# Fireflies-17/Speech-Inpainting

Hardware: AMD Instinct MI355X
Metric: real-time factor (audio-sec/wall-sec) per GPU, 4 s clips @16 kHz, 200 ms mask (higher is better)
Workload: dtype encoder GEMMs and attention products: bf16 MFMA, fp32 accumulate (softmax, LayerNorm, head, arg-max in fp32); vocoder: fp16 MFMA (operands rounded to fp16, saturating), fp32 accumulate, activations stored as fp16; 1 GPU; BASELINE configs[1]: batch=32 x 4 s clips per GPU, 200 ms mask, HuBERT-base + HiFi-GAN V1; step = masked log-mel front-end -> encoder -> arg-max/splice -> vocoder on resident raw clips; global_batch=32, clip_samples=64000, mask_frames=10, parallelism=utterance-sharded x1

## Files before the change

include/si_hip.h:

```cpp
#ifndef SI_HIP_H
#define SI_HIP_H

#include <stddef.h>
#include <stdint.h>

#ifdef __cplusplus
extern "C" {
#endif

#define SI_ABI_VERSION 3

enum {
    SI_OK = 0,
    SI_EINVAL = -1,
    SI_ENOMEM = -2,
    SI_EHIP = -3,
    SI_ESTATE = -4,
    SI_EWEIGHTS = -5
};

enum {
    SI_MATH_F32 = 0,
    SI_MATH_BF16 = 1,
    SI_MATH_BF16X3 = 2,
// ... 118 lines not shown
    const double* dwin;
    const double* time_reg;
} si_sinc_filter;
int si_resample_sinc(si_ctx* ctx, const float* x, const int32_t* n_len, int B, int n_in, const si_sinc_filter* f, int n_out, float* y,
                     si_stream_t stream);

int si_pcm16(si_ctx* ctx, const float* wav, int64_t n, int16_t* out, si_stream_t stream);

int si_hifigan_forward(si_ctx* ctx, const float* mel, int B, int Tm, int stretch, float* wav_out,
                       void* workspace, size_t workspace_bytes, si_stream_t stream);

int si_extend_mel(si_ctx* ctx, const float* mel, int B, int Tm, float* out, si_stream_t stream);

int si_hifigan_forward_varlen(si_ctx* ctx, const float* mel, const int32_t* mel_len, int B, int Tm, int stretch, float* wav_out,
                              void* workspace, size_t workspace_bytes, si_stream_t stream);

int si_mel_frames(int n22);
int si_mel_workspace_bytes(si_ctx* ctx, int B, int N22, size_t* out);
int si_mel_frontend(si_ctx* ctx, const float* wave22, const int32_t* mask_start, const int32_t* mask_end, int normalize,
                    int B, int N22, float* mel_out, void* workspace, size_t workspace_bytes, si_stream_t stream);

int si_mel_frontend_varlen(si_ctx* ctx, const float* wave22, const int32_t* mask_start, const int32_t* mask_end, const int32_t* sample_len,
                           int normalize, int B, int N22, float* mel_out, void* workspace, size_t workspace_bytes, si_stream_t stream);

#define SI_MAX_SPANS 16
typedef struct si_span_table {
    int32_t struct_size;
    int32_t num_clips;
    int32_t num_spans;
    int32_t reserved;
// ... 151 lines not shown
```

speech_inpainting_amd/csrc/api.hip:

```cpp
#include <cmath>
#include <cstdarg>
#include <cstdio>
#include <cstdlib>
#include <cstring>
#include <map>
#include <sstream>
#include <string>
#include <vector>

#include "common.h"

namespace {

struct HostTensor {
    const float* data = nullptr;
    std::vector<long> shape;
    long numel() const { long n = 1; for (long d : shape) n *= d; return n; }
};

struct GemmW {
    size_t w = 0, w_lo = 0, bias = 0;
    int Cin = 0, N = 0, Npad = 0, ntaps = 0, groups = 1, math = 0;
    bool has_bias = false;
};

struct LayerW { GemmW qkv, out, ffn1, ffn2; size_t ln1_g, ln1_b, ln2_g, ln2_b; };
struct ConvW { GemmW g; size_t ln_g = 0, ln_b = 0; };
struct ResW { GemmW c1[SI_MAX_DIL], c2[SI_MAX_DIL]; };

struct Layout {
    size_t total = 0;
    size_t conv0_w, conv0_bias, conv0_g, conv0_b;
    std::vector<ConvW> convs;
    size_t fp_ln_g, fp_ln_b; GemmW proj;
    GemmW pos; size_t enc_ln_g, enc_ln_b;
    std::vector<LayerW> layers;
// ... 209 lines not shown
    L.cb_rnorm = P.floats(d.num_clusters);
    L.mel_ld = si_round_up(d.num_mels, 32);
    const int C0 = d.up_initial_channel;
    L.pre = P.gemm(vm, 1, 7, C0, L.mel_ld, true);
    L.ups.clear(); L.rbs.clear();
    int c = C0;
    for (int i = 0; i < d.num_ups; ++i) {
        const int u = d.up_rates[i], k = d.up_kernels[i], cout = stage_channels(ctx, i);
        L.ups.push_back(P.gemm(vm, 1, (k + u - 1) / u, u * cout, c, true));
        c = cout;
        for (int j = 0; j < d.num_rb; ++j) {
            ResW r;
            for (int n = 0; n < d.num_dil; ++n) {
                r.c1[n] = P.gemm(vm, 1, d.rb_kernels[j], c, c, true);
                if (d.resblock_type != 2) r.c2[n] = P.gemm(vm, 1, d.rb_kernels[j], c, c, true);
            }
            L.rbs.push_back(r);
        }
    }
    L.post_C = c;
    L.post_w = P.floats((size_t)7 * c);
    L.post_b = P.floats(1);
    L.total = P.cur;
    return SI_OK;
}

struct BlobHeader { uint32_t magic, version; uint64_t fingerprint, total; uint64_t reserved; };
constexpr uint32_t BLOB_MAGIC = 0x42574953u;
uint64_t layout_fingerprint(const si_ctx* ctx) {
    uint64_t h = 1469598103934665603ull;
// ... 242 lines not shown
        for (int j = 0; j < d.num_rb; ++j) {
            const ResW& R = L.rbs[(size_t)i * d.num_rb + j];
            const std::string rp = G + "resblocks." + std::to_string(i * d.num_rb + j) + ".";
            for (int n = 0; n < d.num_dil; ++n) {
                if (d.resblock_type == 2) {
                    const std::string a = rp + "convs." + std::to_string(n);
                    if (P.folded(a, {c, c, d.rb_kernels[j]}, 0, w)) P.conv(R.c1[n], w, c, c, d.rb_kernels[j]);
                    P.bias(R.c1[n], a + ".bias", c);
                    continue;
                }
                const std::string a = rp + "convs1." + std::to_string(n), bb = rp + "convs2." + std::to_string(n);
                if (P.folded(a, {c, c, d.rb_kernels[j]}, 0, w)) P.conv(R.c1[n], w, c, c, d.rb_kernels[j]);
                P.bias(R.c1[n], a + ".bias", c);
                if (P.folded(bb, {c, c, d.rb_kernels[j]}, 0, w)) P.conv(R.c2[n], w, c, c, d.rb_kernels[j]);
                P.bias(R.c2[n], bb + ".bias", c);
            }
        }
    }
    if (P.folded(G + "conv_post", {1, c, 7}, 0, w))
        for (int ci = 0; ci < c; ++ci) for (int k = 0; k < 7; ++k) P.fptr(L.post_w)[(size_t)k * L.post_C + ci] = w[(size_t)ci * 7 + k];
    P.copy_floats(L.post_b, G + "conv_post.bias", 1);
    return P.rc;
}

inline size_t align_up(size_t v, size_t a) { return (v + a - 1) / a * a; }

struct Carver {
    char* base; size_t cap; size_t cur = 0; bool ok = true;
    float* floats(size_t n) { return reinterpret_cast<float*>(bytes(n * 4)); }
    char* bytes(size_t n) {
// ... 981 lines not shown
                        if (opr) {
                            q.x = nullptr; q.x16 = in16;
                            if (r16) { q.res = nullptr; q.res16 = y16; q.out = nullptr; }
                            if (o.copy16) { q.out16 = ynext16; q.out16_slope = o.slope16; }
                        }
                        q.alpha = o.alpha; q.accumulate = o.accumulate; q.acc16 = r16 && o.accumulate;
                        return si_launch_tapgemm(ctx, G.math, q, st);
                    };
                    if (d.resblock_type == 2) {
                        if ((rc = residual_conv(R.c1[n], dl, in_slope, y, y16))) return rc;
                    } else {
                        int frc = 1;
                        if (r16 && (fuse_mask & cout)) {
                            const TapGemmParams w1 = gemm_params(ctx, R.c1[n]), w2 = gemm_params(ctx, R.c2[n]);
                            frc = si_launch_respair(ctx, cout, y16, ynext16, w1.w, w2.w, w1.bias, w2.bias, Bc, (int)Lo, rk, dl, o.alpha, o.accumulate, st,
                                                    dLs(i + 1), hLs(i + 1), o.slope16);
                            if (frc < 0) return frc;
                        }
                        if (frc > 0) {
                            float* t = buf[3];
                            TapGemmParams p = stage_conv(R.c1[n], i + 1, Lo, cout, cout, dl);
                            p.x = y; p.out = t; p.pro_slope = in_slope;
                            if (opr) { p.x = nullptr; p.x16 = y16; p.out = nullptr; p.out16 = t16; p.out16_slope = 0.1f; }
                            if ((rc = si_launch_tapgemm(ctx, R.c1[n].math, p, st))) return rc;
                            if ((rc = !opr ? tap32({t, nst}, "stage%d.rb%d.t%d", i, j, n)
                                           : tap32({t16, nst, 2}, d.vocoder_math == SI_MATH_F16 ? "stage%d.rb%d.t%d.f16" : "stage%d.rb%d.t%d.bf16", i, j, n))) return rc;
                            if ((rc = residual_conv(R.c2[n], 1, opr ? 1.f : 0.1f, t, t16))) return rc;
                        }
                    }
                    if ((rc = tap16(ynext16, nst, "stage%d.rb%d.p%d.f16", i, j, n))) return rc;
                    if ((rc = tap32({ynext, nst}, "stage%d.rb%d.p%d", i, j, n))) return rc;
// ... 90 lines not shown
    ctx->fe_dev = dev;
    return SI_OK;
}

size_t mel_ws_bytes(int B, int N22) {
    const long Tm = (N22 + 2 * FE_PAD - FE_NFFT) / FE_HOP + 1;
    if (Tm < 1) return 0;
    return fe_round((size_t)B * 4) + fe_round((size_t)B * Tm * FE_FRAME * 4) + fe_round((size_t)B * Tm * FE_LDSPEC * 4) + 256 +
           fe_round((size_t)2 * B * 4);
}

}

extern "C" {

int si_mel_frames(int n22) { return n22 + 2 * FE_PAD < FE_NFFT ? 0 : (n22 + 2 * FE_PAD - FE_NFFT) / FE_HOP + 1; }

int si_mel_workspace_bytes(si_ctx* ctx, int B, int N22, size_t* out) {
    if (!ctx || !out || B <= 0 || si_mel_frames(N22) < 1) return si_fail(ctx, SI_EINVAL, "si_mel_workspace_bytes: bad argument");
    *out = mel_ws_bytes(B, N22);
    return SI_OK;
}

static int mel_run(si_ctx* ctx, const float* wave22, const int32_t* mask_start, const int32_t* mask_end, int normalize, int B,
                   int N22, float* mel_out, void* workspace, size_t workspace_bytes, si_stream_t stream, const int32_t* host_len,
                   const SiSpans* spans = nullptr);

int si_mel_frontend_spans(si_ctx* ctx, const float* wave22, const si_span_table* spans, const int32_t* sample_len, int normalize,
                          int B, int N22, float* mel_out, void* workspace, size_t workspace_bytes, si_stream_t stream) {
    if (!ctx) return SI_EINVAL;
// ... 410 lines not shown
```

speech_inpainting_amd/csrc/common.h:

```cpp
#pragma once
#include <hip/hip_runtime.h>
#include <stdint.h>

#include "../../include/si_hip.h"

#define SI_HIP_CHECK(expr)                                                                      \
    do {                                                                                        \
        hipError_t _e = (expr);                                                                 \
        if (_e != hipSuccess) return si_fail_hip(ctx, _e, #expr, __FILE__, __LINE__);           \
    } while (0)

int si_fail_hip(si_ctx* ctx, hipError_t e, const char* what, const char* file, int line);
int si_fail(si_ctx* ctx, int code, const char* fmt, ...);
void si_prof_begin(si_ctx* ctx, const char* name, double flops, double bytes, hipStream_t st);
void si_prof_end(si_ctx* ctx, hipStream_t st);
const char* si_prof_shape_name(const char* name, long M, int N, int K);
int si_ensure_dyn_lds(si_ctx* ctx, const void* kern, size_t bytes);
int si_num_cus(si_ctx* ctx);

typedef unsigned short bf16_t;

struct SiVlTile { int b, row0, L; };
#ifdef __HIPCC__
__device__ __forceinline__ SiVlTile si_vl_tile(const int32_t* __restrict__ lens, int B, int step, int t) {
// ... 264 lines not shown
int si_launch_upsample_stream(si_ctx* ctx, const UpsampleParams& p, hipStream_t st);

struct ResPairParams {
    const unsigned short* y16;
    unsigned short* out16;
    const unsigned short* w1;
    const unsigned short* w2;
    const float* b1;
    const float* b2;
    int B, L, k, dil;
    float alpha;
    int accumulate;
    const int32_t* lens; const int32_t* lens_host;
    int total_tiles;
    float out_slope;
};
int si_launch_respair_wide(si_ctx* ctx, int C, const ResPairParams& p, hipStream_t st);
struct ResChainParams {
    const unsigned short* y16;
    unsigned short* out16;
    const unsigned short* w1[3];
    const unsigned short* w2[3];
    const float* b1[3];
    const float* b2[3];
    int B, L, k;
    int dil[3];
    float alpha;
    int accumulate;
    const int32_t* lens; const int32_t* lens_host;
    int total_tiles;
};
int si_launch_reschain(si_ctx* ctx, int C, const ResChainParams& p, hipStream_t st);
int si_launch_respair(si_ctx* ctx, int C, const unsigned short* y16, unsigned short* out16, const void* w1, const void* w2,
                      const float* b1, const float* b2, int B, int L, int k, int dil, float alpha, int accumulate, hipStream_t st,
                      const int32_t* lens = nullptr, const int32_t* lens_host = nullptr, float out_slope = 1.f);

int si_launch_extend_mel(si_ctx* ctx, const float* mel, int B, int D, int Tm, int Tout, int stretch, float* out, int ldo,
                         hipStream_t st, const int32_t* tm_len = nullptr, const int32_t* tout_len = nullptr);
int si_launch_extend_mel_cf(si_ctx* ctx, const float* mel, int B, int D, int Tm, int Tout, float* out, hipStream_t st);
int si_launch_small_conv1d(si_ctx* ctx, const float* x, const float* w, const float* bias, const float* res, float* y, int B, int Cin,
                           int Tin, int Cout, int Tout, int K, int stride, int dil, int pad, int relu_in, int channels_last, hipStream_t st);
int si_launch_f0enc_fused(si_ctx* ctx, const float* weights, const float* f0, int B, int T, float* h_out, int in_width, int out_width, int width,
                          int n_state, int depth, int down_t, int stride_t, int growth, int dk, int dpad, double macs, hipStream_t st);
int si_launch_unit_frontend(si_ctx* ctx, const int64_t* code, int Fc, const int64_t* f0_code, int Fp, const float* spk_emb,
                            const float* emb_c, int Kc, const float* emb_p, int Kp, int E, int B, float* out, hipStream_t st);
int si_launch_conv_post(si_ctx* ctx, const float* x, const float* w , const float* bias, int B, int L, int C, int k,
                        float* wav, hipStream_t st, const unsigned short* x16 = nullptr ,
                        const int32_t* lens = nullptr, const int32_t* lens_host = nullptr);
```

speech_inpainting_amd/csrc/respair.hip:

```cpp
#include <algorithm>
#include <cstdio>
#include <cstdlib>
#include <type_traits>

#include "common.h"

typedef float f32x4 __attribute__((ext_vector_type(4)));
typedef unsigned int u32x4 __attribute__((ext_vector_type(4)));
typedef unsigned int u32x2 __attribute__((ext_vector_type(2)));
typedef _Float16 f16x8 __attribute__((ext_vector_type(8)));
typedef _Float16 f16x4 __attribute__((ext_vector_type(4)));

constexpr int RPN_HALO = 50;

template <int ROWB>
__device__ __forceinline__ int rpn_swz(int row) {
    if constexpr (ROWB == 128) return (row & 7) << 4;
    else return ((row >> 1) & 3) << 4;
}

template <int C, int R1, int WARPS_M, int TPS, bool ACC, bool VL>
__global__ __launch_bounds__(64 * WARPS_M, 2) void respair_kernel(const ResPairParams p) {
    static_assert(R1 == WARPS_M * 64 && (C == 32 || C == 64), "64-row wave tiles over all C channels");
    constexpr int NT = 64 * WARPS_M;
// ... 264 lines not shown
    const int grid = std::min(total, si_num_cus(ctx) * (WARPS_M == 4 ? 2 : 1));
    char name[48];
    snprintf(name, sizeof(name), p.accumulate ? "respair_f16_c%d_acc" : "respair_f16_c%d", C);
    double rows = (double)p.B * p.L;
    if (vl) { rows = 0; for (int b = 0; b < p.B; ++b) rows += p.lens_host[b]; }
    const double elems = rows * C;
    si_prof_begin(ctx, name, 2.0 * 2.0 * elems * C * p.k, elems * (2.0 + 2.0 + (p.accumulate ? 2.0 : 0.0)) + 2.0 * 2.0 * p.k * C * C, st);
    hipLaunchKernelGGL(kern, dim3(grid), dim3(64 * WARPS_M), lds, st, pk);
    si_prof_end(ctx, st);
    SI_HIP_CHECK(hipGetLastError());
    return SI_OK;
}

int si_launch_respair(si_ctx* ctx, int C, const unsigned short* y16, unsigned short* out16, const void* w1, const void* w2,
                      const float* b1, const float* b2, int B, int L, int k, int dil, float alpha, int accumulate, hipStream_t st,
                      const int32_t* lens, const int32_t* lens_host, float out_slope) {
    if ((C != 32 && C != 64 && C != 128 && C != 256) || k < 3 || k > 11 || (k & 1) == 0 || (k - 1) * dil > 50 ||
        ((long)L + 1024) * C * 2 >= (1L << 31)) return 1;
    if (!b1 || !b2) return 1;
    if ((lens == nullptr) != (lens_host == nullptr)) return si_fail(ctx, SI_EINVAL, "respair: ragged batches need the lengths on the device and on the host");
    ResPairParams p{y16, out16, static_cast<const unsigned short*>(w1), static_cast<const unsigned short*>(w2), b1, b2, B, L, k, dil, alpha, accumulate, lens, lens_host, 0, out_slope};
    if (out_slope != 1.f && C < 128) return 1;
    if (C >= 128) return si_launch_respair_wide(ctx, C, p, st);
    return C == 32 ? respair_launch<32, 256, 4, 11>(ctx, p, st) : respair_launch<64, 512, 8, 4>(ctx, p, st);
}
```

speech_inpainting_amd/csrc/respair_wide.hip:

```cpp
#include <algorithm>
#include <cstdio>
#include <cstdlib>

#include "common.h"

typedef float f32x4 __attribute__((ext_vector_type(4)));
typedef unsigned int u32x4 __attribute__((ext_vector_type(4)));
typedef unsigned int u32x2 __attribute__((ext_vector_type(2)));
typedef _Float16 f16x8 __attribute__((ext_vector_type(8)));
typedef _Float16 f16x4 __attribute__((ext_vector_type(4)));

template <int ROWB>
__device__ __forceinline__ int swz16(int row) {
    if constexpr (ROWB >= 256) return (row & 7) << 5;
    else return ((row >> 1) & 3) << 5;
}

#ifdef RPW_TIMELINE
__device__ unsigned long long rpw_tl[2][10];
#define RPW_TL_DECL unsigned long long tl_t = wall_clock64(); unsigned long long tl_acc[6] = {0, 0, 0, 0, 0, 0}; unsigned long long tl_tiles = 0; unsigned long long tl_w = 0, tl_sub[2] = {0, 0};
#define RPW_TL_W0 tl_w = wall_clock64();
#define RPW_TL_W1(q) tl_sub[q] += wall_clock64() - tl_w;
#define RPW_TL(ph) { const unsigned long long n_ = wall_clock64(); tl_acc[ph] += n_ - tl_t; tl_t = n_; }
#define RPW_TL_TILE ++tl_tiles;
// ... 1 lines not shown
extern "C" int si_debug_rpw_timeline(unsigned long long* out, int reset) {
    if (hipMemcpyFromSymbol(out, HIP_SYMBOL(rpw_tl), sizeof(rpw_tl)) != hipSuccess) return -1;
    if (reset) { unsigned long long z[2][10] = {}; if (hipMemcpyToSymbol(HIP_SYMBOL(rpw_tl), z, sizeof(z)) != hipSuccess) return -1; }
    return 0;
}
#else
#define RPW_TL_DECL
#define RPW_TL_W0
#define RPW_TL_W1(q)
#define RPW_TL(ph)
#define RPW_TL_TILE
#define RPW_TL_FLUSH
#endif

constexpr int RPW_HALO = 50;

template <int C, int R1, int WARPS_M, int WARPS_N, int BKW, bool ACC, bool VL>
__global__ __launch_bounds__(64 * WARPS_M * WARPS_N, 2) void respair_wide_kernel(const ResPairParams p) {
    static_assert((WARPS_M * WARPS_N == 8 || WARPS_M * WARPS_N == 4) && R1 == WARPS_M * 64 && C == WARPS_N * 64, "64 x 64 wave tiles");
    static_assert(BKW == 128 || BKW == 64, "weight-slab depth");
    constexpr int NT = 64 * WARPS_M * WARPS_N;
    constexpr int ROWBY = C * 2;
    constexpr int ROWBW = BKW * 2;
    constexpr int ROWBO = C * 4;
    constexpr int CPRY = C / 8, CPRW = BKW / 8;
    constexpr int NCH = C / BKW;
    constexpr int KS = BKW / 32;
    constexpr int YBYTES = (R1 + RPW_HALO) * ROWBY;
    constexpr int WBYTES = C * ROWBW;
    constexpr int WSLOTS = C * CPRW / NT;
    constexpr int YSLOTS = ((R1 + RPW_HALO) * CPRY + NT - 1) / NT;
    constexpr int YRPP = NT / CPRY, WRPP = NT / CPRW;
    static_assert(C * CPRW % NT == 0 && NT % CPRY == 0 && NT % CPRW == 0, "staging maps");
    static_assert(R1 * ROWBO <= YBYTES + 2 * WBYTES, "the output image reuses the operand region (not the biases behind it)");

    __builtin_amdgcn_s_setreg((0 << 11) | (23 << 6) | 1, 1);
    extern __shared__ __attribute__((aligned(16))) char smem[];
    char* const Ys = smem;
    char* const Ws = smem + YBYTES;
    float* const Bs = reinterpret_cast<float*>(smem + YBYTES + 2 * WBYTES);

    const int tid = threadIdx.x, lane = tid & 63, wave = tid >> 6;
    const int r16 = lane & 15, kg = lane >> 4;
    const int wm0 = (wave / WARPS_N) * 64, wn0 = (wave % WARPS_N) * 64;
    const int k = p.k, d = p.dil;
    const int p1 = d * (k - 1) / 2, p2 = (k - 1) / 2;
    const int BMo = R1 - (k - 1);
    const int R0 = R1 + (k - 1) * d;
    const int tiles_x = (p.L + BMo - 1) / BMo;
    const int total = VL ? p.total_tiles : tiles_x * p.B;
    auto tile_of = [&](int t, int& tb, int& tm0, int& tL) {
        if constexpr (VL) { const SiVlTile v = si_vl_tile(p.lens, p.B, BMo, t); tb = v.b; tm0 = v.row0; tL = v.L; }
        else { tb = t / tiles_x; tm0 = (t - tb * tiles_x) * BMo; tL = p.L; }
    };
    const __amdgpu_buffer_rsrc_t w1rsrc = __builtin_amdgcn_make_buffer_rsrc(const_cast<unsigned short*>(p.w1), 0, k * C * C * 2, 0x00020000);
    const __amdgpu_buffer_rsrc_t w2rsrc = __builtin_amdgcn_make_buffer_rsrc(const_cast<unsigned short*>(p.w2), 0, k * C * C * 2, 0x00020000);

    const int NS1 = k * NCH, NS = 2 * NS1;
    const int wc = tid % CPRW, wr0 = tid / CPRW;
    u32x4 rw[WSLOTS];
    auto issueW1 = [&](int s, int i) {
        const bool second = s >= NS1;
        const int q = second ? s - NS1 : s;
        const int tap = q / NCH, ch = q - tap * NCH;
        const int soff = __builtin_amdgcn_readfirstlane((tap * C * C + ch * BKW) * 2);
        const int n = wr0 + i * WRPP;
        rw[i] = __builtin_amdgcn_raw_buffer_load_b128(second ? w2rsrc : w1rsrc, (n * C + 8 * wc) * 2, soff, 0);
    };
    auto issueW = [&](int s) {
#pragma unroll
        for (int i = 0; i < WSLOTS; ++i) issueW1(s, i);
    };
    auto storeW1 = [&](char* dst, int i) {
        const int n = wr0 + i * WRPP;
        *reinterpret_cast<u32x4*>(dst + n * ROWBW + ((wc << 4) ^ swz16<ROWBW>(n))) = rw[i];
    };
    auto storeW = [&](char* dst) {
#pragma unroll
        for (int i = 0; i < WSLOTS; ++i) storeW1(dst, i);
    };
    const int yc = tid % CPRY, yr0 = tid / CPRY;
    u32x4 ry[YSLOTS];
    auto issueY = [&](int t) {
        int tb, tm0, tL;
        tile_of(t, tb, tm0, tL);
        const int trow0 = tm0 - p2 - p1;
        const __amdgpu_buffer_rsrc_t rs = __builtin_amdgcn_make_buffer_rsrc(const_cast<unsigned short*>(p.y16 + (long)tb * p.L * C), 0, tL * C * 2, 0x00020000);
#pragma unroll
        for (int i = 0; i < YSLOTS; ++i)
            ry[i] = __builtin_amdgcn_raw_buffer_load_b128(rs, ((trow0 + yr0 + i * YRPP) * C + 8 * yc) * 2, 0, 0);
    };

    if (tid < C / 2) {
        const int which = tid / (C / 4), c4 = (tid % (C / 4)) * 4;
        *reinterpret_cast<f32x4*>(Bs + which * C + c4) = *reinterpret_cast<const f32x4*>((which ? p.b2 : p.b1) + c4);
    }
    const int preW = (wn0 + r16) * ROWBW + (swz16<ROWBW>(wn0 + r16) ^ (kg << 4));
    issueW(0);
    issueY(blockIdx.x);
    RPW_TL_DECL

  for (int tile = blockIdx.x; tile < total; tile += gridDim.x) {
    const int nxt = tile + (int)gridDim.x < total ? tile + (int)gridDim.x : tile;
    int b, m0, Lb;
    tile_of(tile, b, m0, Lb);
    const int t_row0 = m0 - p2;
    const long seg = (long)b * p.L * C;
    const __amdgpu_buffer_rsrc_t yrsrc = __builtin_amdgcn_make_buffer_rsrc(const_cast<unsigned short*>(p.y16 + seg), 0, Lb * C * 2, 0x00020000);
    const __amdgpu_buffer_rsrc_t orsrc = __builtin_amdgcn_make_buffer_rsrc(p.out16 + seg, 0, Lb * C * 2, 0x00020000);

    storeW(Ws);
    issueW(1);
#pragma unroll
    for (int i = 0; i < YSLOTS; ++i) {
        const int r = yr0 + i * YRPP;
        if ((i + 1) * YRPP <= R1 || r < R0) {
            f16x8 h = __builtin_bit_cast(f16x8, ry[i]);
            h = __builtin_elementwise_max(h, h * (_Float16)0.1f);
            *reinterpret_cast<f16x8*>(Ys + r * ROWBY + ((yc << 4) ^ swz16<ROWBY>(r))) = h;
        }
    }
    __syncthreads();
    RPW_TL(0)

    f32x4 acc[4][4];
    auto init_acc = [&](const float* bias) {
#pragma unroll
        for (int j = 0; j < 4; ++j) {
            const f32x4 bv = *reinterpret_cast<const f32x4*>(bias + wn0 + 16 * j + 4 * kg);
#pragma unroll
            for (int i = 0; i < 4; ++i) acc[i][j] = bv;
        }
    };
    init_acc(Bs);
    auto compute = [&](int roff, int cb16, const char* Wc, auto&& hook) {
        const int r0 = wm0 + r16 + roff;
        const int preY = r0 * ROWBY + (swz16<ROWBY>(r0) ^ (kg << 4));
        auto load = [&](f16x8 (&y)[4], f16x8 (&w)[4], int ks) {
            const char* yp = Ys + (preY ^ (cb16 + ks * 64));
            const char* wp = Wc + (preW ^ (ks * 64));
#pragma unroll
            for (int i = 0; i < 4; ++i) y[i] = *reinterpret_cast<const f16x8*>(yp + i * (16 * ROWBY));
#pragma unroll
            for (int j = 0; j < 4; ++j) w[j] = *reinterpret_cast<const f16x8*>(wp + j * (16 * ROWBW));
        };
        auto mma = [&](const f16x8 (&y)[4], const f16x8 (&w)[4]) {
#pragma unroll
            for (int i = 0; i < 4; ++i)
#pragma unroll
                for (int j = 0; j < 4; ++j) acc[i][j] = __builtin_amdgcn_mfma_f32_16x16x32_f16(w[j], y[i], acc[i][j], 0, 0, 0);
        };
        f16x8 ya[4], wa[4], yb[4], wb[4];
        load(ya, wa, 0);
#pragma unroll
        for (int ks = 0; ks < KS; ks += 2) {
            load(yb, wb, ks + 1);
            __builtin_amdgcn_sched_barrier(0);
            __builtin_amdgcn_s_setprio(1);
            mma(ya, wa);
            __builtin_amdgcn_s_setprio(0);
            __builtin_amdgcn_sched_barrier(0);
            hook(ks);
            if (ks + 2 < KS) load(ya, wa, ks + 2);
            __builtin_amdgcn_sched_barrier(0);
            __builtin_amdgcn_s_setprio(1);
            mma(yb, wb);
            __builtin_amdgcn_s_setprio(0);
            __builtin_amdgcn_sched_barrier(0);
            hook(ks + 1);
        }
    };

    int tap = 0, ch = 0;
    for (int s = 0; s < NS - 1; ++s) {
        const bool second = s >= NS1;
        char* const Wn = Ws + ((s + 1) & 1) * WBYTES;
        static_assert(WSLOTS % KS == 0, "the slab's stores are spread evenly over its k-steps");
        compute(second ? tap : tap * d, ch * (BKW * 2), Ws + (s & 1) * WBYTES, [&](int ks) {
            const int s2 = s + 2 < NS ? s + 2 : NS - 1;
#pragma unroll
            for (int i = 0; i < WSLOTS / KS; ++i) {
                storeW1(Wn, ks * (WSLOTS / KS) + i);
                issueW1(s2, ks * (WSLOTS / KS) + i);
            }
        });
        if (s == NS1 - 1) {
            __syncthreads();
            RPW_TL(1)
#pragma unroll
            for (int ip = 0; ip < 2; ++ip) {
                float inside[2];
#pragma unroll
                for (int u = 0; u < 2; ++u) {
                    const int grow = t_row0 + wm0 + 16 * (2 * ip + u) + r16;
                    inside[u] = (grow >= 0 && grow < Lb) ? 1.f : 0.f;
                }
                const int ms = wm0 + 16 * (2 * ip + (kg & 1)) + r16;
#pragma unroll
                for (int j = 0; j < 4; ++j) {
                    u32x2 pk[2];
#pragma unroll
                    for (int u = 0; u < 2; ++u) {
                        f16x4 hv;
#pragma unroll
                        for (int e = 0; e < 4; ++e) hv[e] = (_Float16)(si_lrelu01(acc[2 * ip + u][j][e]) * inside[u]);
                        pk[u] = __builtin_bit_cast(u32x2, hv);
                    }
#pragma unroll
                    for (int q = 0; q < 2; ++q) {
                        const auto r = __builtin_amdgcn_permlane16_swap(pk[0][q], pk[1][q], false, false);
                        pk[0][q] = r[0]; pk[1][q] = r[1];
                    }
                    const int ch = ((wn0 + 16 * j) >> 3) + (kg >> 1);
                    *reinterpret_cast<u32x4*>(Ys + ms * ROWBY + ((ch << 4) ^ swz16<ROWBY>(ms))) = u32x4{pk[0][0], pk[0][1], pk[1][0], pk[1][1]};
                }
            }
            init_acc(Bs + C);
            RPW_TL(2)
        }
        if (++ch == NCH) { ch = 0; if (++tap == k) tap = 0; }
        __syncthreads();
    }
    if constexpr (!ACC) issueY(nxt);
    __builtin_amdgcn_sched_barrier(0);
    compute(tap, ch * (BKW * 2), Ws + ((NS - 1) & 1) * WBYTES, [](int) {});
    RPW_TL(3)
    constexpr int ORPP = NT / CPRY;
    constexpr int OPASS = R1 / ORPP;
    const int c8 = tid % CPRY, or0 = tid / CPRY;
    u32x4 res[OPASS], prev[ACC ? OPASS : 1];
    int goff[OPASS];
#pragma unroll
    for (int it = 0; it < OPASS; ++it) {
        const int o = or0 + it * ORPP;
        const int grow = m0 + o;
        goff[it] = (o < BMo && grow < Lb) ? (grow * C + 8 * c8) * 2 : (int)0x80000000;
        res[it] = __builtin_amdgcn_raw_buffer_load_b128(yrsrc, goff[it], 0, 0);
        if constexpr (ACC) prev[it] = __builtin_amdgcn_raw_buffer_load_b128(orsrc, goff[it], 0, 0);
    }
    RPW_TL_W0
    __syncthreads();
    RPW_TL_W1(0)
    RPW_TL_W0

#pragma unroll
    for (int i = 0; i < 4; ++i) {
        const int m = wm0 + 16 * i + r16;
#pragma unroll
        for (int j = 0; j < 4; ++j) {
            const int co = ((wn0 + 16 * j) >> 2) + kg;
            *reinterpret_cast<f32x4*>(smem + m * ROWBO + ((co ^ (m & 15)) << 4)) = acc[i][j];
        }
    }
    RPW_TL_W1(1)
    __syncthreads();
    RPW_TL(4)
    issueW(0);
    {
        const bool oact = p.out_slope != 0.f && p.out_slope != 1.f;
#pragma unroll
        for (int it = 0; it < OPASS; ++it) {
            const int o = or0 + it * ORPP;
            const f32x4 a0 = *reinterpret_cast<const f32x4*>(smem + o * ROWBO + (((2 * c8) ^ (o & 15)) << 4));
            const f32x4 a1 = *reinterpret_cast<const f32x4*>(smem + o * ROWBO + (((2 * c8 + 1) ^ (o & 15)) << 4));
            const f16x8 rh = __builtin_bit_cast(f16x8, res[it]);
            f16x8 ph = {};
            if constexpr (ACC) ph = __builtin_bit_cast(f16x8, prev[it]);
            f16x8 out;
#pragma unroll
            for (int e = 0; e < 8; ++e) {
                const float a = e < 4 ? a0[e] : a1[e - 4];
                float v = (a + (float)rh[e]) * p.alpha;
                if constexpr (ACC) v += (float)ph[e];
                if (oact) v = v > 0.f ? v : v * p.out_slope;
                out[e] = (_Float16)v;
            }
            __builtin_amdgcn_raw_buffer_store_b128(__builtin_bit_cast(u32x4, out), orsrc, goff[it], 0, 0);
        }
    }
    if constexpr (ACC) issueY(nxt);
    __syncthreads();
    RPW_TL(5)
    RPW_TL_TILE
  }
  RPW_TL_FLUSH
}

template <int C, int R1, int WARPS_M, int WARPS_N, int BKW>
static int respair_wide_launch(si_ctx* ctx, const ResPairParams& p0, hipStream_t st) {
    const ResPairParams& p = p0;
    const int BMo = R1 - (p.k - 1);
    const size_t lds = (size_t)(R1 + RPW_HALO) * C * 2 + 2 * (size_t)C * BKW * 2 + 2 * (size_t)C * 4;
    const bool vl = p0.lens != nullptr;
    auto kern = vl ? (p.accumulate ? respair_wide_kernel<C, R1, WARPS_M, WARPS_N, BKW, true, true> : respair_wide_kernel<C, R1, WARPS_M, WARPS_N, BKW, false, true>)
                   : (p.accumulate ? respair_wide_kernel<C, R1, WARPS_M, WARPS_N, BKW, true, false> : respair_wide_kernel<C, R1, WARPS_M, WARPS_N, BKW, false, false>);
    if (int rc = si_ensure_dyn_lds(ctx, reinterpret_cast<const void*>(kern), lds)) return rc;
    const int total = vl ? (int)si_vl_tiles(p.lens_host, p.B, BMo) : ((p.L + BMo - 1) / BMo) * p.B;
    if (total <= 0) return SI_OK;
    ResPairParams pk = p0;
    pk.total_tiles = total;
    const int grid = std::min(total, si_num_cus(ctx) * (WARPS_M * WARPS_N == 4 ? 2 : 1));
    char name[48];
    snprintf(name, sizeof(name), p.accumulate ? "respair_f16_c%d_acc" : "respair_f16_c%d", C);
    double rows = (double)p.B * p.L;
    if (vl) { rows = 0; for (int b = 0; b < p.B; ++b) rows += p.lens_host[b]; }
    const double elems = rows * C;
    si_prof_begin(ctx, name, 2.0 * 2.0 * elems * C * p.k, elems * (2.0 + 2.0 + (p.accumulate ? 2.0 : 0.0)) + 2.0 * 2.0 * p.k * C * C, st);
    hipLaunchKernelGGL(kern, dim3(grid), dim3(64 * WARPS_M * WARPS_N), lds, st, pk);
    si_prof_end(ctx, st);
    SI_HIP_CHECK(hipGetLastError());
    return SI_OK;
}

int si_launch_respair_wide(si_ctx* ctx, int C, const ResPairParams& p, hipStream_t st) {
    if (C == 128) return respair_wide_launch<128, 256, 4, 2, 128>(ctx, p, st);
    if (C == 256) return respair_wide_launch<256, 128, 2, 4, 64>(ctx, p, st);
    return 1;
}
```

speech_inpainting_amd/native.py:

```python
from __future__ import annotations

import ctypes as C
import os
from typing import Optional

import numpy as np
import torch

from .arch import HubertArch, VocoderArch

_HERE = os.path.dirname(os.path.abspath(__file__))
LIB_PATH = os.environ.get("SI_HIP_LIB") or os.path.join(_HERE, "libsi_hip.so")

SI_MATH = {"fp32": 0, "f32": 0, "bf16": 1, "bf16x3": 2, "fp16": 3, "f16": 3}
SI_MAX_CONV, SI_MAX_UPS, SI_MAX_RB, SI_MAX_DIL = 8, 8, 4, 4

EXPORTS = ["si_version", "si_create", "si_destroy", "si_last_error", "si_load_weights", "si_alloc_weights",
           "si_weights_device_ptr", "si_weights_check", "si_workspace_bytes", "si_hubert_forward", "si_hubert_forward_padded", "si_hubert_forward_varlen", "si_hubert_extract_features", "si_code_splice", "si_codebook_splice",
           "si_codebook_splice_varlen", "si_hifigan_forward_varlen", "si_mel_frontend_varlen",
           "si_codebook_splice_labels", "si_codebook_metrics", "si_kmeans_assign", "si_mel_metrics", "si_sisdr", "si_unit_frontend",
           "si_f0_encoder_weight_floats", "si_f0_encoder_frames", "si_f0_encoder_workspace_bytes", "si_f0_encoder_forward",
           "si_resample_poly", "si_resample_sinc", "si_pcm16", "si_extend_mel", "si_hifigan_forward", "si_mel_frames", "si_mel_workspace_bytes", "si_mel_frontend", "si_num_frames",
           "si_vocoder_samples", "si_profile_start", "si_profile_filter", "si_profile_stop",
           "si_debug_capture", "si_debug_size",
           "si_hubert_forward_spans", "si_mel_frontend_spans", "si_codebook_splice_spans", "si_codebook_splice_labels_spans",
           "si_codebook_metrics_spans", "si_wave_peak", "si_gather_windows", "si_patch_compose",
           "si_cut_clips", "si_patch_regions", "si_quiet_runs", "si_patch_rate"]
SI_MAX_SPANS = 16


class _F0EncStruct(C.Structure):
    _fields_ = [(n, C.c_int32) for n in ("in_width", "out_width", "width", "n_state", "depth", "down_t", "stride_t", "dilation_growth")]


class F0EncDesc:

    def __init__(self, in_width=1, out_width=128, width=32, depth=4, down_t=4, stride_t=2, dilation_growth=3, m_conv=1.0):
        self.in_width, self.out_width, self.width, self.depth = int(in_width), int(out_width), int(width), int(depth)
        self.down_t, self.stride_t, self.dilation_growth = int(down_t), int(stride_t), int(dilation_growth)
        self.n_state = int(m_conv * width)

    def as_struct(self) -> _F0EncStruct:
# ... 261 lines not shown
    lib.si_mel_frames.argtypes = [i32]
    lib.si_mel_workspace_bytes.argtypes = [vp, i32, i32, C.POINTER(sz)]
    lib.si_mel_frontend.argtypes = [vp, vp, vp, vp, i32, i32, i32, vp, vp, sz, vp]
    lib.si_hubert_forward_spans.argtypes = [vp, vp, C.POINTER(SpanTableStruct), vp, i32, i32, i32, vp, vp, sz, vp]
    lib.si_mel_frontend_spans.argtypes = [vp, vp, C.POINTER(SpanTableStruct), vp, i32, i32, i32, vp, vp, sz, vp]
    lib.si_codebook_splice_spans.argtypes = [vp, vp, i32, i32, vp, vp, i32, vp, i32, vp, vp]
    lib.si_codebook_splice_labels_spans.argtypes = [vp, vp, i32, vp, vp, i32, vp, i32, vp]
    lib.si_codebook_metrics_spans.argtypes = [vp, vp, i32, i32, vp, vp, i32, vp, vp, vp, vp, vp, vp]
    lib.si_wave_peak.argtypes = [vp, vp, C.POINTER(SpanTableStruct), vp, i32, i32, vp, vp]
    lib.si_gather_windows.argtypes = [vp, vp, i32, i32, vp, vp, i32, i32, vp, vp]
    lib.si_patch_compose.argtypes = [vp, vp, C.POINTER(SpanTableStruct), vp, C.POINTER(PatchTableStruct), vp, i32, vp, i32, i32, vp, vp, vp]
    lib.si_cut_clips.argtypes = [vp, vp, i32, vp, vp, i32, i32, vp, vp]
    lib.si_patch_regions.argtypes = [vp, vp, i32, C.POINTER(RegionTableStruct), vp, i32, vp, vp, vp, vp]
    lib.si_quiet_runs.argtypes = [vp, vp, i32, i32, C.c_float, i32, vp, i32, vp, vp]
    lib.si_patch_rate.argtypes = [vp, vp, i32, i32, i32, C.POINTER(RateTableStruct), vp, i32, vp, C.POINTER(SincFilter), vp, vp]
    lib.si_num_frames.argtypes = [vp, i32]
    lib.si_vocoder_samples.argtypes = [vp, i32, i32]
    lib.si_debug_capture.argtypes = [vp, C.c_char_p, vp, C.c_long]
    lib.si_debug_size.argtypes = [vp, C.c_char_p]
    lib.si_debug_size.restype = C.c_long
    lib.si_profile_start.argtypes = [vp, i32]
    lib.si_profile_filter.argtypes = [vp, C.c_char_p]
    lib.si_profile_stop.argtypes = [vp, C.POINTER(ProfileEntry), i32, C.POINTER(i32)]
    for name in EXPORTS:
        if name not in ("si_destroy", "si_last_error", "si_debug_size"):
            getattr(lib, name).restype = i32
    if path is None:
        _lib = lib
    return lib

# ... 533 lines not shown
```

Measured before the change: 11060 x real-time (audio-sec/wall-sec); `value` = whole-job aggregate over n_gpus, `value_per_gpu` = the per-GPU figure the metric names.

## Stream fragment-major resblock weights from registers instead of LDS in wide respair kernel

Adds a fragment-major fp16 weight copy for the 128/256-channel resblock conv pairs, packed at load time, so each wave can load its MFMA B operands straight from global memory into a register ring without staging through LDS. The wide respair kernel changes to one wave per SIMD with 128x64 wave tiles and 8 M-tiles, and uses one block per CU. Activation LDS reads are interleaved with the MFMAs. This removes the LDS weight slabs and their per-slab barriers, at the cost of extra weight memory, higher register pressure and half the resident blocks per CU.

```diff
diff --git a/include/si_hip.h b/include/si_hip.h
--- a/include/si_hip.h
+++ b/include/si_hip.h
@@ -156,6 +156,8 @@
 
 int si_hifigan_forward_varlen(si_ctx* ctx, const float* mel, const int32_t* mel_len, int B, int Tm, int stretch, float* wav_out,
                               void* workspace, size_t workspace_bytes, si_stream_t stream);
+
+int si_respair_wfrag_pack(const uint16_t* src, uint16_t* dst, int k, int C);
 
 int si_mel_frames(int n22);
 int si_mel_workspace_bytes(si_ctx* ctx, int B, int N22, size_t* out);
diff --git a/speech_inpainting_amd/csrc/api.hip b/speech_inpainting_amd/csrc/api.hip
--- a/speech_inpainting_amd/csrc/api.hip
+++ b/speech_inpainting_amd/csrc/api.hip
@@ -20,6 +20,7 @@
 
 struct GemmW {
     size_t w = 0, w_lo = 0, bias = 0;
+    size_t w_frag = 0;
     int Cin = 0, N = 0, Npad = 0, ntaps = 0, groups = 1, math = 0;
     bool has_bias = false;
 };
@@ -259,6 +260,8 @@
             for (int n = 0; n < d.num_dil; ++n) {
                 r.c1[n] = P.gemm(vm, 1, d.rb_kernels[j], c, c, true);
                 if (d.resblock_type != 2) r.c2[n] = P.gemm(vm, 1, d.rb_kernels[j], c, c, true);
+                if (vm == SI_MATH_F16 && d.resblock_type != 2 && (c == 128 || c == 256))
+                    for (GemmW* g : {&r.c1[n], &r.c2[n]}) g->w_frag = P.take((size_t)g->ntaps * c * c * 2);
             }
             L.rbs.push_back(r);
         }
@@ -531,6 +534,11 @@
                 P.bias(R.c1[n], a + ".bias", c);
                 if (P.folded(bb, {c, c, d.rb_kernels[j]}, 0, w)) P.conv(R.c2[n], w, c, c, d.rb_kernels[j]);
                 P.bias(R.c2[n], bb + ".bias", c);
+                for (const GemmW* g : {&R.c1[n], &R.c2[n]})
+                    if (g->w_frag) {
+                        if (g->Npad != c) return si_fail(ctx, SI_EWEIGHTS, "fragment-major copy: %d padded rows for %d channels", g->Npad, c);
+                        si_respair_wfrag_pack(reinterpret_cast<const uint16_t*>(P.out.data() + g->w), reinterpret_cast<uint16_t*>(P.out.data() + g->w_frag), g->ntaps, c);
+                    }
             }
         }
     }
@@ -1542,7 +1550,8 @@
                         if (r16 && (fuse_mask & cout)) {
                             const TapGemmParams w1 = gemm_params(ctx, R.c1[n]), w2 = gemm_params(ctx, R.c2[n]);
                             frc = si_launch_respair(ctx, cout, y16, ynext16, w1.w, w2.w, w1.bias, w2.bias, Bc, (int)Lo, rk, dl, o.alpha, o.accumulate, st,
-                                                    dLs(i + 1), hLs(i + 1), o.slope16);
+                                                    dLs(i + 1), hLs(i + 1), o.slope16,
+                                                    R.c1[n].w_frag ? ctx->wdev + R.c1[n].w_frag : nullptr, R.c2[n].w_frag ? ctx->wdev + R.c2[n].w_frag : nullptr);
                             if (frc < 0) return frc;
                         }
                         if (frc > 0) {
@@ -1663,6 +1672,14 @@
 
 extern "C" {
 
+int si_respair_wfrag_pack(const uint16_t* src, uint16_t* dst, int k, int C) {
+    if (!src || !dst || k < 1 || C < 32 || C % 32) return si_fail(nullptr, SI_EINVAL, "si_respair_wfrag_pack: bad argument");
+    for (int tap = 0; tap < k; ++tap)
+        for (int n = 0; n < C; ++n)
+            for (int ci = 0; ci < C; ++ci) dst[si_wfrag_index(C, tap, n, ci)] = src[((size_t)tap * C + n) * C + ci];
+    return SI_OK;
+}
+
 int si_mel_frames(int n22) { return n22 + 2 * FE_PAD < FE_NFFT ? 0 : (n22 + 2 * FE_PAD - FE_NFFT) / FE_HOP + 1; }
 
 int si_mel_workspace_bytes(si_ctx* ctx, int B, int N22, size_t* out) {
diff --git a/speech_inpainting_amd/csrc/common.h b/speech_inpainting_amd/csrc/common.h
--- a/speech_inpainting_amd/csrc/common.h
+++ b/speech_inpainting_amd/csrc/common.h
@@ -302,7 +302,13 @@
     const int32_t* lens; const int32_t* lens_host;
     int total_tiles;
     float out_slope;
-};
+    const unsigned short* w1f;
+    const unsigned short* w2f;
+};
+inline size_t si_wfrag_index(int C, int tap, int n, int ci) {
+    const int ks = ci >> 5, lane = (((ci >> 3) & 3) << 4) | (n & 15);
+    return ((((size_t)tap * (C / 32) + ks) * (C / 16) + (n >> 4)) * 64 + lane) * 8 + (ci & 7);
+}
 int si_launch_respair_wide(si_ctx* ctx, int C, const ResPairParams& p, hipStream_t st);
 struct ResChainParams {
     const unsigned short* y16;
@@ -321,7 +327,8 @@
 int si_launch_reschain(si_ctx* ctx, int C, const ResChainParams& p, hipStream_t st);
 int si_launch_respair(si_ctx* ctx, int C, const unsigned short* y16, unsigned short* out16, const void* w1, const void* w2,
                       const float* b1, const float* b2, int B, int L, int k, int dil, float alpha, int accumulate, hipStream_t st,
-                      const int32_t* lens = nullptr, const int32_t* lens_host = nullptr, float out_slope = 1.f);
+                      const int32_t* lens = nullptr, const int32_t* lens_host = nullptr, float out_slope = 1.f,
+                      const void* w1f = nullptr, const void* w2f = nullptr);
 
 int si_launch_extend_mel(si_ctx* ctx, const float* mel, int B, int D, int Tm, int Tout, int stretch, float* out, int ldo,
                          hipStream_t st, const int32_t* tm_len = nullptr, const int32_t* tout_len = nullptr);
diff --git a/speech_inpainting_amd/csrc/respair.hip b/speech_inpainting_amd/csrc/respair.hip
--- a/speech_inpainting_amd/csrc/respair.hip
+++ b/speech_inpainting_amd/csrc/respair.hip
@@ -302,12 +302,13 @@
 
 int si_launch_respair(si_ctx* ctx, int C, const unsigned short* y16, unsigned short* out16, const void* w1, const void* w2,
                       const float* b1, const float* b2, int B, int L, int k, int dil, float alpha, int accumulate, hipStream_t st,
-                      const int32_t* lens, const int32_t* lens_host, float out_slope) {
+                      const int32_t* lens, const int32_t* lens_host, float out_slope, const void* w1f, const void* w2f) {
     if ((C != 32 && C != 64 && C != 128 && C != 256) || k < 3 || k > 11 || (k & 1) == 0 || (k - 1) * dil > 50 ||
         ((long)L + 1024) * C * 2 >= (1L << 31)) return 1;
     if (!b1 || !b2) return 1;
     if ((lens == nullptr) != (lens_host == nullptr)) return si_fail(ctx, SI_EINVAL, "respair: ragged batches need the lengths on the device and on the host");
-    ResPairParams p{y16, out16, static_cast<const unsigned short*>(w1), static_cast<const unsigned short*>(w2), b1, b2, B, L, k, dil, alpha, accumulate, lens, lens_host, 0, out_slope};
+    ResPairParams p{y16, out16, static_cast<const unsigned short*>(w1), static_cast<const unsigned short*>(w2), b1, b2, B, L, k, dil, alpha, accumulate, lens, lens_host, 0, out_slope,
+                    static_cast<const unsigned short*>(w1f), static_cast<const unsigned short*>(w2f)};
     if (out_slope != 1.f && C < 128) return 1;
     if (C >= 128) return si_launch_respair_wide(ctx, C, p, st);
     return C == 32 ? respair_launch<32, 256, 4, 11>(ctx, p, st) : respair_launch<64, 512, 8, 4>(ctx, p, st);
diff --git a/speech_inpainting_amd/csrc/respair_wide.hip b/speech_inpainting_amd/csrc/respair_wide.hip
--- a/speech_inpainting_amd/csrc/respair_wide.hip
+++ b/speech_inpainting_amd/csrc/respair_wide.hip
@@ -1,6 +1,7 @@
 #include <algorithm>
 #include <cstdio>
 #include <cstdlib>
+#include <type_traits>
 
 #include "common.h"
 
@@ -39,35 +40,33 @@
 #endif
 
 constexpr int RPW_HALO = 50;
-
-template <int C, int R1, int WARPS_M, int WARPS_N, int BKW, bool ACC, bool VL>
-__global__ __launch_bounds__(64 * WARPS_M * WARPS_N, 2) void respair_wide_kernel(const ResPairParams p) {
-    static_assert((WARPS_M * WARPS_N == 8 || WARPS_M * WARPS_N == 4) && R1 == WARPS_M * 64 && C == WARPS_N * 64, "64 x 64 wave tiles");
-    static_assert(BKW == 128 || BKW == 64, "weight-slab depth");
-    constexpr int NT = 64 * WARPS_M * WARPS_N;
+constexpr int RPW_WRING = 4;
+
+template <int C, int R1, int WARPS_M, int WARPS_N, bool ACC, bool VL>
+__global__ __launch_bounds__(256, 1) void respair_wide_kernel(const ResPairParams p) {
+    static_assert(WARPS_M * WARPS_N == 4 && R1 == WARPS_M * 128 && C == WARPS_N * 64, "128 x 64 wave tiles, one wave per SIMD");
+    constexpr int NT = 256;
+    constexpr int MT = 8;
     constexpr int ROWBY = C * 2;
-    constexpr int ROWBW = BKW * 2;
     constexpr int ROWBO = C * 4;
-    constexpr int CPRY = C / 8, CPRW = BKW / 8;
-    constexpr int NCH = C / BKW;
-    constexpr int KS = BKW / 32;
+    constexpr int CPRY = C / 8;
+    constexpr int KST = C / 32;
+    constexpr int WKB = (C / 16) * 1024;
+    constexpr int WR = RPW_WRING;
     constexpr int YBYTES = (R1 + RPW_HALO) * ROWBY;
-    constexpr int WBYTES = C * ROWBW;
-    constexpr int WSLOTS = C * CPRW / NT;
+    constexpr int LBYTES = YBYTES > R1 * ROWBO ? YBYTES : R1 * ROWBO;
     constexpr int YSLOTS = ((R1 + RPW_HALO) * CPRY + NT - 1) / NT;
-    constexpr int YRPP = NT / CPRY, WRPP = NT / CPRW;
-    static_assert(C * CPRW % NT == 0 && NT % CPRY == 0 && NT % CPRW == 0, "staging maps");
-    static_assert(R1 * ROWBO <= YBYTES + 2 * WBYTES, "the output image reuses the operand region (not the biases behind it)");
+    constexpr int YRPP = NT / CPRY;
+    static_assert(NT % CPRY == 0 && KST % WR == 0 && KST % 2 == 0, "staging map; the ring and the fragment double buffer close per tap");
 
     __builtin_amdgcn_s_setreg((0 << 11) | (23 << 6) | 1, 1);
     extern __shared__ __attribute__((aligned(16))) char smem[];
     char* const Ys = smem;
-    char* const Ws = smem + YBYTES;
-    float* const Bs = reinterpret_cast<float*>(smem + YBYTES + 2 * WBYTES);
+    float* const Bs = reinterpret_cast<float*>(smem + LBYTES);
 
     const int tid = threadIdx.x, lane = tid & 63, wave = tid >> 6;
     const int r16 = lane & 15, kg = lane >> 4;
-    const int wm0 = (wave / WARPS_N) * 64, wn0 = (wave % WARPS_N) * 64;
+    const int wm0 = (wave / WARPS_N) * 128, wn0 = (wave % WARPS_N) * 64;
     const int k = p.k, d = p.dil;
     const int p1 = d * (k - 1) / 2, p2 = (k - 1) / 2;
     const int BMo = R1 - (k - 1);
@@ -78,35 +77,23 @@
         if constexpr (VL) { const SiVlTile v = si_vl_tile(p.lens, p.B, BMo, t); tb = v.b; tm0 = v.row0; tL = v.L; }
         else { tb = t / tiles_x; tm0 = (t - tb * tiles_x) * BMo; tL = p.L; }
     };
-    const __amdgpu_buffer_rsrc_t w1rsrc = __builtin_amdgcn_make_buffer_rsrc(const_cast<unsigned short*>(p.w1), 0, k * C * C * 2, 0x00020000);
-    const __amdgpu_buffer_rsrc_t w2rsrc = __builtin_amdgcn_make_buffer_rsrc(const_cast<unsigned short*>(p.w2), 0, k * C * C * 2, 0x00020000);
-
-    const int NS1 = k * NCH, NS = 2 * NS1;
-    const int wc = tid % CPRW, wr0 = tid / CPRW;
-    u32x4 rw[WSLOTS];
-    auto issueW1 = [&](int s, int i) {
-        const bool second = s >= NS1;
-        const int q = second ? s - NS1 : s;
-        const int tap = q / NCH, ch = q - tap * NCH;
-        const int soff = __builtin_amdgcn_readfirstlane((tap * C * C + ch * BKW) * 2);
-        const int n = wr0 + i * WRPP;
-        rw[i] = __builtin_amdgcn_raw_buffer_load_b128(second ? w2rsrc : w1rsrc, (n * C + 8 * wc) * 2, soff, 0);
-    };
-    auto issueW = [&](int s) {
-#pragma unroll
-        for (int i = 0; i < WSLOTS; ++i) issueW1(s, i);
-    };
-    auto storeW1 = [&](char* dst, int i) {
-        const int n = wr0 + i * WRPP;
-        *reinterpret_cast<u32x4*>(dst + n * ROWBW + ((wc << 4) ^ swz16<ROWBW>(n))) = rw[i];
-    };
-    auto storeW = [&](char* dst) {
-#pragma unroll
-        for (int i = 0; i < WSLOTS; ++i) storeW1(dst, i);
+    const __amdgpu_buffer_rsrc_t w1rsrc = __builtin_amdgcn_make_buffer_rsrc(const_cast<unsigned short*>(p.w1f), 0, k * C * C * 2, 0x00020000);
+    const __amdgpu_buffer_rsrc_t w2rsrc = __builtin_amdgcn_make_buffer_rsrc(const_cast<unsigned short*>(p.w2f), 0, k * C * C * 2, 0x00020000);
+
+    const int wlane = (wn0 >> 4) * 1024 + lane * 16;
+    u32x4 wr[WR][4];
+    auto issueW = [&](int slot, int j, bool second, int soff) __attribute__((always_inline)) {
+        wr[slot][j] = __builtin_amdgcn_raw_buffer_load_b128(second ? w2rsrc : w1rsrc, wlane + j * 1024, soff, 0);
+    };
+    auto fillW = [&]() __attribute__((always_inline)) {
+#pragma unroll
+        for (int s = 0; s < WR; ++s)
+#pragma unroll
+            for (int j = 0; j < 4; ++j) issueW(s, j, false, s * WKB);
     };
     const int yc = tid % CPRY, yr0 = tid / CPRY;
     u32x4 ry[YSLOTS];
-    auto issueY = [&](int t) {
+    auto issueY = [&](int t) __attribute__((always_inline)) {
         int tb, tm0, tL;
         tile_of(t, tb, tm0, tL);
         const int trow0 = tm0 - p2 - p1;
@@ -120,8 +107,7 @@
         const int which = tid / (C / 4), c4 = (tid % (C / 4)) * 4;
         *reinterpret_cast<f32x4*>(Bs + which * C + c4) = *reinterpret_cast<const f32x4*>((which ? p.b2 : p.b1) + c4);
     }
-    const int preW = (wn0 + r16) * ROWBW + (swz16<ROWBW>(wn0 + r16) ^ (kg << 4));
-    issueW(0);
+    fillW();
     issueY(blockIdx.x);
     RPW_TL_DECL
 
@@ -134,8 +120,6 @@
     const __amdgpu_buffer_rsrc_t yrsrc = __builtin_amdgcn_make_buffer_rsrc(const_cast<unsigned short*>(p.y16 + seg), 0, Lb * C * 2, 0x00020000);
     const __amdgpu_buffer_rsrc_t orsrc = __builtin_amdgcn_make_buffer_rsrc(p.out16 + seg, 0, Lb * C * 2, 0x00020000);
 
-    storeW(Ws);
-    issueW(1);
 #pragma unroll
     for (int i = 0; i < YSLOTS; ++i) {
         const int r = yr0 + i * YRPP;
@@ -148,72 +132,73 @@
     __syncthreads();
     RPW_TL(0)
 
-    f32x4 acc[4][4];
-    auto init_acc = [&](const float* bias) {
+    f32x4 acc[MT][4];
+    auto init_acc = [&](const float* bias) __attribute__((always_inline)) {
 #pragma unroll
         for (int j = 0; j < 4; ++j) {
             const f32x4 bv = *reinterpret_cast<const f32x4*>(bias + wn0 + 16 * j + 4 * kg);
 #pragma unroll
-            for (int i = 0; i < 4; ++i) acc[i][j] = bv;
-        }
-    };
+            for (int i = 0; i < MT; ++i) acc[i][j] = bv;
+        }
+    };
+    f16x8 ya[MT], yb[MT];
+    auto preYof = [&](int roff) {
+        const int r0 = wm0 + r16 + roff;
+        return r0 * ROWBY + (swz16<ROWBY>(r0) ^ (kg << 4));
+    };
+    auto loadY1 = [&](f16x8 (&y)[MT], int pre, int ks, int i) __attribute__((always_inline)) {
+        y[i] = *reinterpret_cast<const f16x8*>(Ys + (pre ^ (ks * 64)) + i * (16 * ROWBY));
+    };
+    auto loadY = [&](f16x8 (&y)[MT], int pre) __attribute__((always_inline)) {
+#pragma unroll
+        for (int i = 0; i < MT; ++i) loadY1(y, pre, 0, i);
+    };
+    auto kstep = [&](const f16x8 (&cur)[MT], f16x8 (&nxt)[MT], int slot, bool next, int preX, int ksX, bool wl, bool wsec, int wsoff) __attribute__((always_inline)) {
+#pragma unroll
+        for (int j = 0; j < 4; ++j) {
+            const f16x8 wv = __builtin_bit_cast(f16x8, wr[slot][j]);
+#pragma unroll
+            for (int i = 0; i < MT; ++i) {
+                acc[i][j] = __builtin_amdgcn_mfma_f32_16x16x32_f16(wv, cur[i], acc[i][j], 0, 0, 0);
+                const int m = j * MT + i;
+                if (next && m % 3 == 0 && m / 3 < MT) {
+                    loadY1(nxt, preX, ksX, m / 3);
+                    __builtin_amdgcn_sched_barrier(0);
+                }
+            }
+            if (wl) issueW(slot, j, wsec, wsoff);
+            __builtin_amdgcn_sched_barrier(0);
+        }
+    };
+    auto run_tap = [&](auto last_c, int preC, int preN, bool secA, int soffA, bool secB, int soffB, auto&& at_tail) __attribute__((always_inline)) {
+        constexpr bool LAST = decltype(last_c)::value;
+#pragma unroll
+        for (int ks = 0; ks < KST; ++ks) {
+            const bool inside = ks + WR < KST;
+            const bool next = !(LAST && ks == KST - 1);
+            const bool wl = inside || !LAST;
+            const int wsoff = (inside ? soffA : soffB) + ((ks + WR) % KST) * WKB;
+            const int preX = ks + 1 < KST ? preC : preN, ksX = ks + 1 < KST ? ks + 1 : 0;
+            if (ks == KST - WR) { at_tail(); __builtin_amdgcn_sched_barrier(0); }
+            if (ks & 1) kstep(yb, ya, ks % WR, next, preX, ksX, wl, inside ? secA : secB, wsoff);
+            else kstep(ya, yb, ks % WR, next, preX, ksX, wl, inside ? secA : secB, wsoff);
+        }
+    };
+
     init_acc(Bs);
-    auto compute = [&](int roff, int cb16, const char* Wc, auto&& hook) {
-        const int r0 = wm0 + r16 + roff;
-        const int preY = r0 * ROWBY + (swz16<ROWBY>(r0) ^ (kg << 4));
-        auto load = [&](f16x8 (&y)[4], f16x8 (&w)[4], int ks) {
-            const char* yp = Ys + (preY ^ (cb16 + ks * 64));
-            const char* wp = Wc + (preW ^ (ks * 64));
-#pragma unroll
-            for (int i = 0; i < 4; ++i) y[i] = *reinterpret_cast<const f16x8*>(yp + i * (16 * ROWBY));
-#pragma unroll
-            for (int j = 0; j < 4; ++j) w[j] = *reinterpret_cast<const f16x8*>(wp + j * (16 * ROWBW));
-        };
-        auto mma = [&](const f16x8 (&y)[4], const f16x8 (&w)[4]) {
-#pragma unroll
-            for (int i = 0; i < 4; ++i)
-#pragma unroll
-                for (int j = 0; j < 4; ++j) acc[i][j] = __builtin_amdgcn_mfma_f32_16x16x32_f16(w[j], y[i], acc[i][j], 0, 0, 0);
-        };
-        f16x8 ya[4], wa[4], yb[4], wb[4];
-        load(ya, wa, 0);
-#pragma unroll
-        for (int ks = 0; ks < KS; ks += 2) {
-            load(yb, wb, ks + 1);
-            __builtin_amdgcn_sched_barrier(0);
-            __builtin_amdgcn_s_setprio(1);
-            mma(ya, wa);
-            __builtin_amdgcn_s_setprio(0);
-            __builtin_amdgcn_sched_barrier(0);
-            hook(ks);
-            if (ks + 2 < KS) load(ya, wa, ks + 2);
-            __builtin_amdgcn_sched_barrier(0);
-            __builtin_amdgcn_s_setprio(1);
-            mma(yb, wb);
-            __builtin_amdgcn_s_setprio(0);
-            __builtin_amdgcn_sched_barrier(0);
-            hook(ks + 1);
-        }
-    };
-
-    int tap = 0, ch = 0;
-    for (int s = 0; s < NS - 1; ++s) {
-        const bool second = s >= NS1;
-        char* const Wn = Ws + ((s + 1) & 1) * WBYTES;
-        static_assert(WSLOTS % KS == 0, "the slab's stores are spread evenly over its k-steps");
-        compute(second ? tap : tap * d, ch * (BKW * 2), Ws + (s & 1) * WBYTES, [&](int ks) {
-            const int s2 = s + 2 < NS ? s + 2 : NS - 1;
-#pragma unroll
-            for (int i = 0; i < WSLOTS / KS; ++i) {
-                storeW1(Wn, ks * (WSLOTS / KS) + i);
-                issueW1(s2, ks * (WSLOTS / KS) + i);
-            }
-        });
-        if (s == NS1 - 1) {
+    loadY(ya, preYof(0));
+    for (int tt = 0; tt < 2 * k - 1; ++tt) {
+        const bool sec = tt >= k, secn = tt + 1 >= k;
+        const int tc = sec ? tt - k : tt, tcn = secn ? tt + 1 - k : tt + 1;
+        const int preC = preYof(sec ? tc : tc * d);
+        const int preN = tt == k - 1 ? preC : preYof(secn ? tcn : tcn * d);
+        const int soffA = __builtin_amdgcn_readfirstlane(tc * KST * WKB), soffB = __builtin_amdgcn_readfirstlane(tcn * KST * WKB);
+        run_tap(std::false_type{}, preC, preN, sec, soffA, secn, soffB, [] {});
+        if (tt == k - 1) {
             __syncthreads();
             RPW_TL(1)
 #pragma unroll
-            for (int ip = 0; ip < 2; ++ip) {
+            for (int ip = 0; ip < MT / 2; ++ip) {
                 float inside[2];
 #pragma unroll
                 for (int u = 0; u < 2; ++u) {
@@ -242,13 +227,15 @@
             }
             init_acc(Bs + C);
             RPW_TL(2)
-        }
-        if (++ch == NCH) { ch = 0; if (++tap == k) tap = 0; }
-        __syncthreads();
-    }
-    if constexpr (!ACC) issueY(nxt);
-    __builtin_amdgcn_sched_barrier(0);
-    compute(tap, ch * (BKW * 2), Ws + ((NS - 1) & 1) * WBYTES, [](int) {});
+            __syncthreads();
+            loadY(ya, preYof(0));
+        }
+    }
+    {
+        const int preC = preYof(k - 1);
+        const int soffA = __builtin_amdgcn_readfirstlane((k - 1) * KST * WKB);
+        run_tap(std::true_type{}, preC, preC, true, soffA, true, soffA, [&]() __attribute__((always_inline)) { if constexpr (!ACC) issueY(nxt); });
+    }
     RPW_TL(3)
     constexpr int ORPP = NT / CPRY;
     constexpr int OPASS = R1 / ORPP;
@@ -269,7 +256,7 @@
     RPW_TL_W0
 
 #pragma unroll
-    for (int i = 0; i < 4; ++i) {
+    for (int i = 0; i < MT; ++i) {
         const int m = wm0 + 16 * i + r16;
 #pragma unroll
         for (int j = 0; j < 4; ++j) {
@@ -280,7 +267,7 @@
     RPW_TL_W1(1)
     __syncthreads();
     RPW_TL(4)
-    issueW(0);
+    fillW();
     {
         const bool oact = p.out_slope != 0.f && p.out_slope != 1.f;
 #pragma unroll
@@ -311,34 +298,35 @@
   RPW_TL_FLUSH
 }
 
-template <int C, int R1, int WARPS_M, int WARPS_N, int BKW>
+template <int C, int R1, int WARPS_M, int WARPS_N>
 static int respair_wide_launch(si_ctx* ctx, const ResPairParams& p0, hipStream_t st) {
     const ResPairParams& p = p0;
+    if (!p.w1f || !p.w2f) return si_fail(ctx, SI_EINVAL, "respair_wide: C = %d needs the fragment-major weight copies", C);
     const int BMo = R1 - (p.k - 1);
-    const size_t lds = (size_t)(R1 + RPW_HALO) * C * 2 + 2 * (size_t)C * BKW * 2 + 2 * (size_t)C * 4;
+    const size_t lds = std::max((size_t)(R1 + RPW_HALO) * C * 2, (size_t)R1 * C * 4) + 2 * (size_t)C * 4;
     const bool vl = p0.lens != nullptr;
-    auto kern = vl ? (p.accumulate ? respair_wide_kernel<C, R1, WARPS_M, WARPS_N, BKW, true, true> : respair_wide_kernel<C, R1, WARPS_M, WARPS_N, BKW, false, true>)
-                   : (p.accumulate ? respair_wide_kernel<C, R1, WARPS_M, WARPS_N, BKW, true, false> : respair_wide_kernel<C, R1, WARPS_M, WARPS_N, BKW, false, false>);
+    auto kern = vl ? (p.accumulate ? respair_wide_kernel<C, R1, WARPS_M, WARPS_N, true, true> : respair_wide_kernel<C, R1, WARPS_M, WARPS_N, false, true>)
+                   : (p.accumulate ? respair_wide_kernel<C, R1, WARPS_M, WARPS_N, true, false> : respair_wide_kernel<C, R1, WARPS_M, WARPS_N, false, false>);
     if (int rc = si_ensure_dyn_lds(ctx, reinterpret_cast<const void*>(kern), lds)) return rc;
     const int total = vl ? (int)si_vl_tiles(p.lens_host, p.B, BMo) : ((p.L + BMo - 1) / BMo) * p.B;
     if (total <= 0) return SI_OK;
     ResPairParams pk = p0;
     pk.total_tiles = total;
-    const int grid = std::min(total, si_num_cus(ctx) * (WARPS_M * WARPS_N == 4 ? 2 : 1));
+    const int grid = std::min(total, si_num_cus(ctx));
     char name[48];
     snprintf(name, sizeof(name), p.accumulate ? "respair_f16_c%d_acc" : "respair_f16_c%d", C);
     double rows = (double)p.B * p.L;
     if (vl) { rows = 0; for (int b = 0; b < p.B; ++b) rows += p.lens_host[b]; }
     const double elems = rows * C;
     si_prof_begin(ctx, name, 2.0 * 2.0 * elems * C * p.k, elems * (2.0 + 2.0 + (p.accumulate ? 2.0 : 0.0)) + 2.0 * 2.0 * p.k * C * C, st);
-    hipLaunchKernelGGL(kern, dim3(grid), dim3(64 * WARPS_M * WARPS_N), lds, st, pk);
+    hipLaunchKernelGGL(kern, dim3(grid), dim3(256), lds, st, pk);
     si_prof_end(ctx, st);
     SI_HIP_CHECK(hipGetLastError());
     return SI_OK;
 }
 
 int si_launch_respair_wide(si_ctx* ctx, int C, const ResPairParams& p, hipStream_t st) {
-    if (C == 128) return respair_wide_launch<128, 256, 4, 2, 128>(ctx, p, st);
-    if (C == 256) return respair_wide_launch<256, 128, 2, 4, 64>(ctx, p, st);
+    if (C == 128) return respair_wide_launch<128, 256, 2, 2>(ctx, p, st);
+    if (C == 256) return respair_wide_launch<256, 128, 1, 4>(ctx, p, st);
     return 1;
 }
diff --git a/speech_inpainting_amd/native.py b/speech_inpainting_amd/native.py
--- a/speech_inpainting_amd/native.py
+++ b/speech_inpainting_amd/native.py
@@ -25,7 +25,7 @@
            "si_debug_capture", "si_debug_size",
            "si_hubert_forward_spans", "si_mel_frontend_spans", "si_codebook_splice_spans", "si_codebook_splice_labels_spans",
            "si_codebook_metrics_spans", "si_wave_peak", "si_gather_windows", "si_patch_compose",
-           "si_cut_clips", "si_patch_regions", "si_quiet_runs", "si_patch_rate"]
+           "si_cut_clips", "si_patch_regions", "si_quiet_runs", "si_patch_rate", "si_respair_wfrag_pack"]
 SI_MAX_SPANS = 16
 
 
@@ -317,6 +317,7 @@
     lib.si_patch_regions.argtypes = [vp, vp, i32, C.POINTER(RegionTableStruct), vp, i32, vp, vp, vp, vp]
     lib.si_quiet_runs.argtypes = [vp, vp, i32, i32, C.c_float, i32, vp, i32, vp, vp]
     lib.si_patch_rate.argtypes = [vp, vp, i32, i32, i32, C.POINTER(RateTableStruct), vp, i32, vp, C.POINTER(SincFilter), vp, vp]
+    lib.si_respair_wfrag_pack.argtypes = [vp, vp, i32, i32]
     lib.si_num_frames.argtypes = [vp, i32]
     lib.si_vocoder_samples.argtypes = [vp, i32, i32]
     lib.si_debug_capture.argtypes = [vp, C.c_char_p, vp, C.c_long]
```

Result: faster. 11410 x real-time (audio-sec/wall-sec); `value` = whole-job aggregate over n_gpus, `value_per_gpu` = the per-GPU figure the metric names, median of 6 (+3.2%).
